# finleygou/GS-MARL

Measured on NVIDIA B200. Metric: agent-steps/sec (graph obs+reward+cost) at 1/2/4/8 B200; % HBM roofline, higher is better.
Workload: dtype f32

## Files before the change

gs_marl_b200/csrc/gsm_kernels_wide.cuh:

```cuda
#pragma once
#include "gsm_kernels_spec.cuh"
#include "gsm_bulk.cuh"

namespace gsm {

constexpr int kWideThreads = 128;
__host__ __device__ constexpr int wide_pow2(int v) { int p = 1; while (p < v) p <<= 1; return p; }

template <typename T, int N, int E>
struct WideConsts {
  T size[E];
  T mass[N], mass_inv[N], accel[N], maxsp[N];
  int32_t eflag[E];
};

#ifndef GSM_WIDE_BLOCKS
#define GSM_WIDE_BLOCKS 7
#endif
template <typename T> struct WideMinBlocks { static constexpr int value = sizeof(T) == 4 ? GSM_WIDE_BLOCKS : 1; };

__device__ __forceinline__ float softplus1(float x) {
  float y, l;
  asm("ex2.approx.ftz.f32 %0, %1;" : "=f"(y) : "f"(-fabsf(x) * 1.4426950408889634f));
  asm("lg2.approx.ftz.f32 %0, %1;" : "=f"(l) : "f"(1.0f + y));
  return fmaxf(x, 0.f) + 0.6931471805599453f * l;
}
__device__ __forceinline__ double softplus1(double x) { return fmax(x, 0.0) + r_log1p(r_exp(-fabs(x))); }

__device__ __forceinline__ int keep(int v) { return __shfl_sync(0xffffffffu, v, threadIdx.x & 31); }
__device__ __forceinline__ unsigned keep(unsigned v) { return __shfl_sync(0xffffffffu, v, threadIdx.x & 31); }
__device__ __forceinline__ float keep(float v) { return __shfl_sync(0xffffffffu, v, threadIdx.x & 31); }
__device__ __forceinline__ double keep(double v) { return __shfl_sync(0xffffffffu, v, threadIdx.x & 31); }

__device__ __forceinline__ void sts(unsigned a, unsigned v) { asm volatile("st.shared.u32 [%0], %1;" :: "r"(a), "r"(v) : "memory"); }
__device__ __forceinline__ void sts(unsigned a, int v) { asm volatile("st.shared.u32 [%0], %1;" :: "r"(a), "r"(v) : "memory"); }
__device__ __forceinline__ void sts(unsigned a, float v) { asm volatile("st.shared.f32 [%0], %1;" :: "r"(a), "f"(v) : "memory"); }
__device__ __forceinline__ void sts(unsigned a, double v) { asm volatile("st.shared.f64 [%0], %1;" :: "r"(a), "d"(v) : "memory"); }
__device__ __forceinline__ void sts2(unsigned a, float x, float y) { asm volatile("st.shared.v2.f32 [%0], {%1, %2};" :: "r"(a), "f"(x), "f"(y) : "memory"); }
__device__ __forceinline__ void sts2(unsigned a, double x, double y) { asm volatile("st.shared.v2.f64 [%0], {%1, %2};" :: "r"(a), "d"(x), "d"(y) : "memory"); }
__device__ __forceinline__ void sts4(unsigned a, float x, float y, float z, float w) {
  asm volatile("st.shared.v4.f32 [%0], {%1, %2, %3, %4};" :: "r"(a), "f"(x), "f"(y), "f"(z), "f"(w) : "memory");
}
__device__ __forceinline__ void sts4(unsigned a, double x, double y, double z, double w) { sts2(a, x, y); sts2(a + 16, z, w); }
__device__ __forceinline__ void lds4(unsigned a, float& x, float& y, float& z, float& w) {
  asm volatile("ld.shared.v4.f32 {%0, %1, %2, %3}, [%4];" : "=f"(x), "=f"(y), "=f"(z), "=f"(w) : "r"(a) : "memory");
}
__device__ __forceinline__ void lds4(unsigned a, double& x, double& y, double& z, double& w) {
  asm volatile("ld.shared.v2.f64 {%0, %1}, [%2];" : "=d"(x), "=d"(y) : "r"(a) : "memory");
  asm volatile("ld.shared.v2.f64 {%0, %1}, [%2];" : "=d"(z), "=d"(w) : "r"(a + 16) : "memory");
}
__device__ __forceinline__ void sts_if(bool on, unsigned a, unsigned v) {
  asm volatile("{ .reg .pred q; setp.ne.u32 q, %2, 0; @q st.shared.u32 [%0], %1; }" :: "r"(a), "r"(v), "r"((unsigned)on) : "memory");
}
__device__ __forceinline__ void sts2_if(bool on, unsigned a, float x, float y) {
  asm volatile("{ .reg .pred q; setp.ne.u32 q, %3, 0; @q st.shared.v2.f32 [%0], {%1, %2}; }" :: "r"(a), "f"(x), "f"(y), "r"((unsigned)on) : "memory");
}
__device__ __forceinline__ void sts2_if(bool on, unsigned a, double x, double y) {
  asm volatile("{ .reg .pred q; setp.ne.u32 q, %3, 0; @q st.shared.v2.f64 [%0], {%1, %2}; }" :: "r"(a), "d"(x), "d"(y), "r"((unsigned)on) : "memory");
}
__device__ __forceinline__ unsigned selp(bool c, unsigned a, unsigned b) {
  unsigned r;
  asm("{ .reg .pred q; setp.ne.u32 q, %3, 0; selp.b32 %0, %1, %2, q; }" : "=r"(r) : "r"(a), "r"(b), "r"((unsigned)c));
  return r;
}
__device__ __forceinline__ float div_eager(float a, float b) {
  float r; asm volatile("div.approx.f32 %0, %1, %2;" : "=f"(r) : "f"(a), "f"(b)); return r;
}
__device__ __forceinline__ double div_eager(double a, double b) { return a / b; }
__device__ __forceinline__ float4 lds16(unsigned a) {
  float4 v; asm volatile("ld.shared.v4.f32 {%0, %1, %2, %3}, [%4];" : "=f"(v.x), "=f"(v.y), "=f"(v.z), "=f"(v.w) : "r"(a) : "memory"); return v;
}

template <typename T>
__device__ __forceinline__ T shfl_xor(T v, int m) { return __shfl_xor_sync(0xffffffffu, v, m); }

template <typename T> struct __align__(16) WideEnt { T x, y, vx, vy; };

struct WideSmem {
  unsigned feat, idx, obs, cnt, adj, cost, rew, asg, buf;
  unsigned ent, warp;
};
__host__ __device__ constexpr WideSmem wide_smem_layout(int rb, int N, int E, int K, int EPW) {
  WideSmem w{};
  unsigned o = 0;
  w.feat = o; o += (unsigned)(EPW * N * K * GSM_NBR_FEAT_DIM * rb);
  w.idx = o; o += ((unsigned)(EPW * N * K * 4) + 15u) & ~15u;
  w.obs = o; o += (unsigned)(EPW * N * GSM_OBS_DIM * rb);
  w.cnt = o; o += (unsigned)(EPW * N * 4);
  w.adj = o; o += (unsigned)(EPW * N * 4);
  w.cost = o; o += (unsigned)(EPW * N * rb);
  w.rew = o; o += (unsigned)(EPW * N * rb);
  w.asg = o; o += (unsigned)(EPW * N * 4);
  w.buf = (o + 15u) & ~15u;
  w.ent = 2 * w.buf;
  w.warp = w.ent + (unsigned)(EPW * E * 4 * rb);
  return w;
}
__host__ __device__ constexpr size_t wide_smem_bytes(int rb, int N, int E, int K, int EPW) {
  return (size_t)(kWideThreads / 32) * wide_smem_layout(rb, N, E, K, EPW).warp;
}

template <typename T, int N, int L, int MODE, int KT>
__global__ void __launch_bounds__(kWideThreads, WideMinBlocks<T>::value)
env_wide_kernel(const __grid_constant__ KParams<T> p, const int n_steps,
                const __grid_constant__ StepStrides ss,
                const __grid_constant__ WideConsts<T, N, N + L> wc,
                const __grid_constant__ WideSmem lay_rt) {
  constexpr int E = N + L, M = E - 1, GW = wide_pow2(M), EPW = 32 / GW;
  constexpr bool OBS = MODE == 1;
  constexpr bool BF = MODE == 2;
  constexpr unsigned FULL = 0xffffffffu;
  constexpr int RB = (int)sizeof(T);
  constexpr int RS4 = EPW * N * 4, RST = EPW * N * RB;
  constexpr int PS = (RS4 % 16 == 0 && RST % 16 == 0) ? 16 : 8;
  constexpr int PC4 = RS4 / PS, PCT = RST / PS, NPIECE = 3 * PC4 + 2 * PCT;
  constexpr bool ROLE_OK = NPIECE <= 32;
  static_assert(GW <= 32 && E <= 32, "an env must fit in one warp, adjacency in one word");
  static_assert(L >= N && 2 * N <= GW + 1 && N >= 3, "goal i is landmark i, held by lane N-1+i; lanes 0..2 stage scalars");
  static_assert(RS4 % 8 == 0 && RST % 8 == 0, "per-warp scalar blocks leave in 8- or 16-byte pieces");
  static_assert(EPW * N * M * 4 / 16 <= 64 && EPW * N * GSM_OBS_DIM * RB / 16 <= 64, "idx / obs blocks leave in <= 2 passes");
  typedef Arith<T> A;
  typedef WideEnt<T> Ent;
  typedef float4 V;
  extern __shared__ __align__(128) unsigned char wsm[];
  const int K = KT > 0 ? KT : p.K;
  const WideSmem lay = KT > 0 ? wide_smem_layout((int)sizeof(T), N, N + L, KT > 0 ? KT : 1, 32 / wide_pow2(N + L - 1)) : lay_rt;
  const int lane = keep((int)(threadIdx.x & 31)), warp = threadIdx.x >> 5;
  const int grp = lane / GW, j = lane % GW, shift = grp * GW;
  const int env_w0 = keep((int)(((int64_t)blockIdx.x * (kWideThreads / 32) + warp) * EPW));
  bool active = env_w0 + grp < p.n_envs;
  if (OBS && p.mask != nullptr && active) active = p.mask[(int64_t)(env_w0 + grp) * p.mask_stride] != 0;
  const int env = active ? env_w0 + grp : 0;
  const bool has = M == GW ? true : j < M;
  const bool own = j < N;
  const int ja = own ? j : 0;
  const unsigned act_bits = __ballot_sync(FULL, active);
  const bool bulk = ROLE_OK && act_bits == FULL && ((EPW * N * K * 4) & 15) == 0 &&
      ((((uintptr_t)p.obs | (uintptr_t)p.nbr_idx | (uintptr_t)p.nbr_feat | (uintptr_t)p.nbr_cnt | (uintptr_t)p.adj |
         (uintptr_t)p.assign | (uintptr_t)p.reward | (uintptr_t)p.cost | (uintptr_t)ss.obs | (uintptr_t)ss.nbr_idx |
         (uintptr_t)ss.nbr_feat | (uintptr_t)ss.nbr_cnt | (uintptr_t)ss.adj | (uintptr_t)ss.assign |
         (uintptr_t)ss.reward | (uintptr_t)ss.cost) & 15) == 0);

  constexpr unsigned ES = (unsigned)sizeof(Ent);
  const unsigned sa_w = keep(smem_u32(wsm) + (unsigned)warp * lay.warp);
  const unsigned sa_ent = keep(smem_u32(wsm) + (unsigned)warp * lay.warp + lay.ent + (unsigned)(grp * E) * ES);

  const int e_hi = has ? j + 1 : 0;
  const int fl_o = wc.eflag[e_hi];
  const T size_o = keep(wc.size[e_hi]), type_o = keep((T)(fl_o >> 1));
  const unsigned lfl = keep((unsigned)((has && (wc.eflag[0] & 1) && (fl_o & 1)) ? 1u : 0u) |
                            ((has && (e_hi < N || (p.cost_obstacles && (fl_o >> 1) == GSM_ENT_OBSTACLE))) ? 2u : 0u) |
                            (((has && p.own_goal_always && j >= N - 1 && j < 2 * N - 1) ? (unsigned)(j - (N - 1) + 1) : 0u) << 8));
  const bool cpair = lfl & 1u, colc = lfl & 2u;
  const int goal_i = (int)(lfl >> 8) - 1;

  T mx = 0, my = 0, mvx = 0, mvy = 0;
  if (active) {
    const T* a = p.agent_state + ((int64_t)env * N + ja) * 4;
    mx = a[0]; my = a[1]; mvx = a[2]; mvy = a[3];
  }
  if (own) sts4(sa_ent + (unsigned)j * ES, mx, my, mvx, mvy);
  if (has && j + 1 >= N) {
    T lx = 0, ly = 0;
    if (active) { const T* l = p.lm_pos + ((int64_t)env * L + (j + 1 - N)) * 2; lx = l[0]; ly = l[1]; }
    sts4(sa_ent + (unsigned)(j + 1) * ES, lx, ly, (T)0, (T)0);
  }
  int t_now = active ? p.t[env] : 0;
  const bool auto_reset = MODE == 2 && p.auto_reset != 0;
  const T accel_m = keep(wc.accel[ja]), mass_m = keep(wc.mass[ja]), massinv_m = keep(wc.mass_inv[ja]), maxsp_m = keep(wc.maxsp[ja]);

  const unsigned char* b_act = (const unsigned char*)p.actions;
  unsigned char* b_obs = (unsigned char*)p.obs;
  unsigned char* b_idx = (unsigned char*)p.nbr_idx;
  unsigned char* b_feat = (unsigned char*)p.nbr_feat;
  unsigned char* b_done = (unsigned char*)p.done;
  const unsigned wrow0 = (unsigned)env_w0 * N;
  unsigned char* c_role = nullptr;
  int64_t role_stride = ss.nbr_cnt;
  {
    const int q = lane;
    if (q < PC4) c_role = (unsigned char*)p.nbr_cnt + wrow0 * 4u + q * PS;
    else if (q < 2 * PC4) { c_role = (unsigned char*)p.adj + wrow0 * 4u + (q - PC4) * PS; if (RB != 4) role_stride = ss.adj; }
    else if (q < 2 * PC4 + PCT) { c_role = (unsigned char*)p.cost + wrow0 * (unsigned)RB + (q - 2 * PC4) * PS; if (RB != 4) role_stride = ss.cost; }
    else if (q < 2 * PC4 + 2 * PCT) { c_role = (unsigned char*)p.reward + wrow0 * (unsigned)RB + (q - 2 * PC4 - PCT) * PS; if (RB != 4) role_stride = ss.reward; }
    else if (q < NPIECE) { c_role = (unsigned char*)p.assign + wrow0 * 4u + (q - 2 * PC4 - 2 * PCT) * PS; if (RB != 4) role_stride = ss.assign; }
  }
  const bool role_on = lane < NPIECE && (!OBS || lane < 2 * PC4 || lane >= 2 * PC4 + 2 * PCT);
  if (own) {
    sts(sa_w + lay.asg + (unsigned)(grp * N + j) * 4u, j);
    sts(sa_w + lay.buf + lay.asg + (unsigned)(grp * N + j) * 4u, j);
  }

  const bool discrete = p.action_mode == GSM_ACT_DISCRETE;
  const unsigned act_off = keep(discrete ? ((unsigned)env * N + ja) * 4u : ((unsigned)env * N + ja) * 2u * (unsigned)RB);
  const unsigned n_idx = (lay.obs - lay.idx) / 16, n_obs = (lay.cnt - lay.obs) / 16;
  const unsigned off_idx = keep(wrow0 * (unsigned)(K * 4) + (unsigned)lane * 16u), off_obs = keep(wrow0 * (unsigned)(GSM_OBS_DIM * RB) + (unsigned)lane * 16u);
  const unsigned off_done = keep((unsigned)env * N + (unsigned)ja);
  int act_next = 0;
  T actx_next = 0, acty_next = 0;
  if (!OBS) {
    if (discrete) act_next = *(const int32_t*)(b_act + act_off);
    else { actx_next = ((const T*)(b_act + act_off))[0]; acty_next = ((const T*)(b_act + act_off))[1]; }
  }
  __syncwarp();

  T fox = 0, foy = 0;
  bool pro = !OBS;
  int step = 0;
  unsigned sb = sa_w;
  int sb_delta = (int)lay.buf;
  const unsigned o_feat = keep((unsigned)(grp * N * K) * (unsigned)(GSM_NBR_FEAT_DIM * RB));
  const unsigned o_idx = keep(lay.idx + (unsigned)(grp * N * K) * 4u);
  const unsigned o_sc = keep(lay.cnt + (unsigned)(j < 3 ? j : 0) * (unsigned)RS4 + (unsigned)(grp * N) * 4u);
  const unsigned o_obs = keep(lay.obs + (unsigned)grp * (unsigned)(N * GSM_OBS_DIM * RB));
  const auto segment_end = [&]() {
    int s = n_steps;
    if (MODE == 2 && auto_reset) {
      const int left = __reduce_min_sync(FULL, active ? p.episode_length - t_now : INT_MAX);
      s = step + max(1, min(left, n_steps - step));
    }
    return s;
  };
  int stop = segment_end();
  while (step < n_steps) {
   for (;;) {
    if (!OBS && !pro) {
      T ux = actx_next, uy = acty_next;
      if (discrete) {
        const int a = act_next;
        ux = 0; uy = 0;
        if (a >= 0 && a < p.n_actions) { ux = p.discrete_u[a][0]; uy = p.discrete_u[a][1]; }
      }
      if (step + 1 < n_steps) b_act += ss.actions;
      if (discrete) act_next = *(const int32_t*)(b_act + act_off);
      else { actx_next = ((const T*)(b_act + act_off))[0]; acty_next = ((const T*)(b_act + act_off))[1]; }
      const T fx = accel_m * ux + fox, fy = accel_m * uy + foy;
      T nvx = mvx * p.one_minus_damp, nvy = mvy * p.one_minus_damp;
      nvx = nvx + A::div_const(fx, mass_m, massinv_m) * p.dt;
      nvy = nvy + A::div_const(fy, mass_m, massinv_m) * p.dt;
      if (maxsp_m > (T)0) {
        const T sp = A::sqrt(nvx * nvx + nvy * nvy);
        if (sp > maxsp_m) { nvx = A::div(nvx, sp) * maxsp_m; nvy = A::div(nvy, sp) * maxsp_m; }
      }
      mvx = nvx; mvy = nvy;
      mx = mx + nvx * p.dt; my = my + nvy * p.dt;
      t_now += 1;
      if (own) sts4(sa_ent + (unsigned)j * ES, mx, my, mvx, mvy);
      __syncwarp();
    }
    const bool st_on = !pro;
    const unsigned a_feat = sb + o_feat, a_idx = sb + o_idx, a_sc = sb + o_sc, sobs = sb + o_obs;
    if (st_on && bulk && lane == 0) bulk_wait_read<1>();

    T fcx[N], fcy[N];
    T gxs = 0, gys = 0, gd = 0;
    bool anyc = false;
#pragma unroll
    for (int i = 0; i < N; i++) {
      const int e = e_hi - (j < i ? 1 : 0);
      Ent si, so;
      lds4(sa_ent + (unsigned)i * ES, si.x, si.y, si.vx, si.vy);
      lds4(sa_ent + (unsigned)e * ES, so.x, so.y, so.vx, so.vy);
      const T dx = so.x - si.x, dy = so.y - si.y;
      const T dist = A::sqrt(dx * dx + dy * dy);
      const T dmin = wc.size[i] + size_o;
      const bool nb = (has && dist < p.Rs) || goal_i == i;
      const bool col = colc && dist < dmin;
      const unsigned bits = (__ballot_sync(FULL, nb) >> shift) & low_mask(GW);
      const unsigned cbits = (__ballot_sync(FULL, col) >> shift) & low_mask(GW);
      int cnt = __popc(bits);
      const int rank = __popc(bits & low_mask(j));
      const int pos = nb ? rank : cnt + (j - rank);
      if (BF) {
        const bool row_on = st_on && has && (KT >= M || pos < K);
        sts_if(row_on, a_idx + (unsigned)pos * 4u + (unsigned)(i * K * 4), (unsigned)(nb ? e : -1));
        const unsigned f = a_feat + (unsigned)pos * (unsigned)(GSM_NBR_FEAT_DIM * RB) + (unsigned)(i * K * GSM_NBR_FEAT_DIM * RB);
        const T z = (T)0;
        sts2_if(row_on, f, nb ? dx : z, nb ? dy : z);
        sts2_if(row_on, f + 2 * RB, nb ? so.vx - si.vx : z, nb ? so.vy - si.vy : z);
        sts2_if(row_on, f + 4 * RB, nb ? dist : z, nb ? type_o : z);
      } else if (has && pos < K && st_on) {
        sts(a_idx + (unsigned)pos * 4u + (unsigned)(i * K * 4), nb ? e : -1);
        const unsigned f = a_feat + (unsigned)pos * (unsigned)(GSM_NBR_FEAT_DIM * RB) + (unsigned)(i * K * GSM_NBR_FEAT_DIM * RB);
        const T z = (T)0;
        if (nb) { sts2(f, dx, dy); sts2(f + 2 * RB, so.vx - si.vx, so.vy - si.vy); sts2(f + 4 * RB, dist, type_o); }
        else { sts2(f, z, z); sts2(f + 2 * RB, z, z); sts2(f + 4 * RB, z, z); }
      }
      if (cnt > K) cnt = K;
      const unsigned ebits = (bits & low_mask(i)) | ((bits & ~low_mask(i)) << 1);
      if (BF && RB == 4) {
        const unsigned v = selp(j == 0, (unsigned)cnt, selp(j == 1, ebits, __float_as_uint((float)__popc(cbits))));
        sts_if(st_on && j < 3, a_sc + (unsigned)(i * 4), v);
      } else if (st_on && j < 3) {
        const unsigned ao = (unsigned)(grp * N + i);
        if (RB == 4) {
          const unsigned v = j == 0 ? (unsigned)cnt : (j == 1 ? ebits : __float_as_uint((float)__popc(cbits)));
          if (!OBS || j < 2) sts(a_sc + (unsigned)(i * 4), v);
        } else {
          if (j == 0) sts(sb + lay.cnt + ao * 4u, cnt);
          else if (j == 1) sts(sb + lay.adj + ao * 4u, ebits);
          else if (!OBS) sts(sb + lay.cost + ao * (unsigned)RB, (T)__popc(cbits));
        }
      }
      if (j == N - 1 + i) { gxs = dx; gys = dy; gd = dist; }
      if (BF) {
        const T x = A::div_const(-(dist - dmin), p.km, p.km_inv);
        const bool term = cpair && !(Prec<T>::kCut && x < (T)(-kFarCut));
        const T pen = softplus1(x) * p.km;
        const T qx = div_eager(p.cf * (-dx), dist), qy = div_eager(p.cf * (-dy), dist);
        fcx[i] = term ? qx * pen : (T)0;
        fcy[i] = term ? qy * pen : (T)0;
        anyc = anyc || term;
      } else if (!OBS) {
        fcx[i] = 0; fcy[i] = 0;
        if (cpair) {
          const T x = A::div_const(-(dist - dmin), p.km, p.km_inv);
          if (!(Prec<T>::kCut && x < (T)(-kFarCut))) {
            const T pen = softplus1(x) * p.km;
            fcx[i] = A::div(p.cf * (-dx), dist) * pen;
            fcy[i] = A::div(p.cf * (-dy), dist) * pen;
            anyc = true;
          }
        }
      }
    }
    if (!OBS && (pro || step + 1 < n_steps)) {
      fox = 0; foy = 0;
      if (__any_sync(FULL, anyc)) {
#pragma unroll
        for (int m = GW / 2; m >= 1; m >>= 1) {
#pragma unroll
          for (int i = 0; i < N; i++) { fcx[i] = fcx[i] + shfl_xor(fcx[i], m); fcy[i] = fcy[i] + shfl_xor(fcy[i], m); }
        }
#pragma unroll
        for (int i = 0; i < N; i++) if (ja == i) { fox = fcx[i]; foy = fcy[i]; }
      }
    }

    if (st_on) {
      if (own) { sts2(sobs + (unsigned)j * (GSM_OBS_DIM * RB), mvx, mvy); sts2(sobs + (unsigned)j * (GSM_OBS_DIM * RB) + 2 * RB, mx, my); }
      T rs = ((T)0 - p.w_dist * gd) + (gd < p.goal_tol ? p.w_goal : (T)0);
      if (p.share_reward && !OBS) {
        T s = shfl(FULL, rs, shift + N - 1);
#pragma unroll
        for (int k = 1; k < N; k++) s = s + shfl(FULL, rs, shift + N - 1 + k);
        rs = s / (T)N;
      }
      if (j >= N - 1 && j < 2 * N - 1) {
        const unsigned ao = (unsigned)(j - (N - 1));
        sts2(sobs + ao * (GSM_OBS_DIM * RB) + 4 * RB, gxs, gys);
        if (!OBS) sts(sb + lay.rew + ((unsigned)grp * N + ao) * (unsigned)RB, rs);
      }
      if (!OBS && own && active) b_done[off_done] = (uint8_t)(t_now >= p.episode_length);
      if (bulk) {
        fence_async_smem();
        __syncwarp();
        if (lane == 0) {
          asm volatile("cp.async.bulk.global.shared::cta.bulk_group [%0], [%1], %2;"
                       :: "l"(b_feat + wrow0 * (unsigned)(K * GSM_NBR_FEAT_DIM * RB)), "r"(sb), "r"(lay.idx) : "memory");
          bulk_commit();
        }
        V* const g_idx = (V*)(b_idx + off_idx);
        V* const g_obs = (V*)(b_obs + off_obs);
        const unsigned s_idx = sb + lay.idx + (unsigned)lane * 16u, s_obs = sb + lay.obs + (unsigned)lane * 16u;
        if (lane < n_idx) g_idx[0] = lds16(s_idx);
        if (lane + 32 < n_idx) g_idx[32] = lds16(s_idx + 512);
        if (lane < n_obs) g_obs[0] = lds16(s_obs);
        if (lane + 32 < n_obs) g_obs[32] = lds16(s_obs + 512);
        if (role_on) {
          if (PS == 16) *(V*)c_role = lds16(sb + lay.cnt + (unsigned)lane * 16u);
          else {
            float2 v8;
            asm volatile("ld.shared.v2.f32 {%0, %1}, [%2];" : "=f"(v8.x), "=f"(v8.y) : "r"(sb + lay.cnt + (unsigned)lane * 8u) : "memory");
            *(float2*)c_role = v8;
          }
        }
      } else {
        __syncwarp();
        auto copy_words = [&](unsigned char* g, unsigned soff, unsigned bytes) {
          const unsigned wpe = bytes / (4 * EPW);
          for (unsigned q = lane; q < bytes / 4; q += 32)
            if ((act_bits >> ((q / wpe) * GW)) & 1u) {
              unsigned v; asm volatile("ld.shared.u32 %0, [%1];" : "=r"(v) : "r"(sb + soff + q * 4u) : "memory");
              ((uint32_t*)g)[q] = v;
            }
        };
        copy_words(b_feat + wrow0 * (unsigned)(K * GSM_NBR_FEAT_DIM * RB), lay.feat, lay.idx - lay.feat);
        copy_words(b_idx + wrow0 * (unsigned)(K * 4), lay.idx, (unsigned)(EPW * N * K * 4));
        copy_words(b_obs + wrow0 * (unsigned)(GSM_OBS_DIM * RB), lay.obs, lay.cnt - lay.obs);
        copy_words((unsigned char*)p.nbr_cnt + (int64_t)step * ss.nbr_cnt + wrow0 * 4u, lay.cnt, RS4);
        copy_words((unsigned char*)p.adj + (int64_t)step * ss.adj + wrow0 * 4u, lay.adj, RS4);
        copy_words((unsigned char*)p.assign + (int64_t)step * ss.assign + wrow0 * 4u, lay.asg, RS4);
        if (!OBS) {
          copy_words((unsigned char*)p.reward + (int64_t)step * ss.reward + wrow0 * (unsigned)RB, lay.rew, RST);
          copy_words((unsigned char*)p.cost + (int64_t)step * ss.cost + wrow0 * (unsigned)RB, lay.cost, RST);
        }
        __syncwarp();
      }
    }
    if (OBS) break;
    if (pro) { pro = false; continue; }
    b_obs += ss.obs; b_idx += ss.nbr_idx; b_feat += ss.nbr_feat; b_done += ss.done;
    c_role += role_stride;
    sb += sb_delta;
    sb_delta = -sb_delta;
    step++;
    if (step >= stop) break;
   }
   if (OBS) break;
   if (MODE == 2 && auto_reset) {
     const bool fin = active && t_now >= p.episode_length;
     if (__any_sync(FULL, fin)) {
       __syncwarp();
       int ep = 0;
       if (fin) {
         const uint64_t genv = (uint64_t)(p.env_offset + env);
         ep = p.episode[env];
#pragma unroll 1
         for (int e = j; e < E; e += GW) {
           double dx, dy;
           spawn_draw_inline(genv, ep, e, p.seed, p.ext[wc.eflag[e] >> 1], dx, dy);
           const T x = (T)dx, y = (T)dy;
           sts4(sa_ent + (unsigned)e * ES, x, y, (T)0, (T)0);
           if (e < N) { mx = x; my = y; }
           else { T* l = p.lm_pos + ((int64_t)env * L + (e - N)) * 2; l[0] = x; l[1] = y; }
         }
         mvx = 0; mvy = 0;
         t_now = 0;
       }
       __syncwarp();
       if (fin && j == 0) p.episode[env] = ep + 1;
       __syncwarp();
       pro = step < n_steps;
       stop = segment_end();
     }
   }
  }
  if (bulk && lane == 0) bulk_wait_read<0>();

  if (!OBS && active) {
    if (own) {
      T* a = p.agent_state + ((int64_t)env * N + j) * 4;
      st2<T>(a, mx, my); st2<T>(a + 2, mvx, mvy);
    }
    if (j == 0) p.t[env] = t_now;
  }
}

}
```

Measured before the change: 16.46 billion.

## Use packed f32x2 arithmetic and streaming cache hints in the BF wide-kernel path

In the BF mode, the velocity and position integration, pairwise deltas, contact-force computation (paired softplus over agents) and the shuffle reductions are rewritten with packed f32x2 add/mul/fma PTX and a scaled rcp-based vector divide. This aims to halve the FP32 instruction count in this path. Global output stores now use evict-first and streaming cache hints, so write-once data is less likely to pollute L2. The divide is now approximate and rounding may change slightly, and the new path needs hardware that supports f32x2 instructions.

```diff
diff --git a/gs_marl_b200/csrc/gsm_kernels_wide.cuh b/gs_marl_b200/csrc/gsm_kernels_wide.cuh
--- a/gs_marl_b200/csrc/gsm_kernels_wide.cuh
+++ b/gs_marl_b200/csrc/gsm_kernels_wide.cuh
@@ -63,10 +63,60 @@
   asm("{ .reg .pred q; setp.ne.u32 q, %3, 0; selp.b32 %0, %1, %2, q; }" : "=r"(r) : "r"(a), "r"(b), "r"((unsigned)c));
   return r;
 }
-__device__ __forceinline__ float div_eager(float a, float b) {
-  float r; asm volatile("div.approx.f32 %0, %1, %2;" : "=f"(r) : "f"(a), "f"(b)); return r;
-}
-__device__ __forceinline__ double div_eager(double a, double b) { return a / b; }
+
+__device__ __forceinline__ float2 bc2(float s) { return make_float2(s, s); }
+__device__ __forceinline__ double2 bc2(double s) { return make_double2(s, s); }
+__device__ __forceinline__ float2 add2(float2 a, float2 b) {
+  float2 r;
+  asm("{ .reg .b64 a, b, d; mov.b64 a, {%2, %3}; mov.b64 b, {%4, %5}; add.rn.f32x2 d, a, b; mov.b64 {%0, %1}, d; }"
+      : "=f"(r.x), "=f"(r.y) : "f"(a.x), "f"(a.y), "f"(b.x), "f"(b.y));
+  return r;
+}
+__device__ __forceinline__ float2 sub2(float2 a, float2 b) {
+  float2 r;
+  asm("{ .reg .b64 a, b, d; mov.b64 a, {%2, %3}; mov.b64 b, {%4, %5}; sub.rn.f32x2 d, a, b; mov.b64 {%0, %1}, d; }"
+      : "=f"(r.x), "=f"(r.y) : "f"(a.x), "f"(a.y), "f"(b.x), "f"(b.y));
+  return r;
+}
+__device__ __forceinline__ float2 mul2(float2 a, float2 b) {
+  float2 r;
+  asm("{ .reg .b64 a, b, d; mov.b64 a, {%2, %3}; mov.b64 b, {%4, %5}; mul.rn.f32x2 d, a, b; mov.b64 {%0, %1}, d; }"
+      : "=f"(r.x), "=f"(r.y) : "f"(a.x), "f"(a.y), "f"(b.x), "f"(b.y));
+  return r;
+}
+__device__ __forceinline__ float2 fma2(float2 a, float2 b, float2 c) {
+  float2 r;
+  asm("{ .reg .b64 a, b, c, d; mov.b64 a, {%2, %3}; mov.b64 b, {%4, %5}; mov.b64 c, {%6, %7}; fma.rn.f32x2 d, a, b, c; mov.b64 {%0, %1}, d; }"
+      : "=f"(r.x), "=f"(r.y) : "f"(a.x), "f"(a.y), "f"(b.x), "f"(b.y), "f"(c.x), "f"(c.y));
+  return r;
+}
+__device__ __forceinline__ double2 add2(double2 a, double2 b) { return make_double2(a.x + b.x, a.y + b.y); }
+__device__ __forceinline__ double2 sub2(double2 a, double2 b) { return make_double2(a.x - b.x, a.y - b.y); }
+__device__ __forceinline__ double2 mul2(double2 a, double2 b) { return make_double2(a.x * b.x, a.y * b.y); }
+__device__ __forceinline__ double2 fma2(double2 a, double2 b, double2 c) { return make_double2(a.x * b.x + c.x, a.y * b.y + c.y); }
+__device__ __forceinline__ float2 div2(float2 a, float b) {
+  float2 r;
+  asm("{ .reg .pred p; .reg .f32 b, t; .reg .b64 a, d;\n\t"
+      "mov.b64 a, {%2, %3}; abs.f32 t, %4; setp.lt.f32 p, t, 0f00800000; selp.f32 t, 0f4B800000, 0f3F800000, p;\n\t"
+      "mul.rn.f32 b, %4, t; mov.b64 d, {t, t}; mul.rn.f32x2 a, a, d;\n\t"
+      "rcp.approx.ftz.f32 t, b; mov.b64 d, {t, t}; mul.rn.f32x2 d, a, d; mov.b64 {%0, %1}, d; }"
+      : "=f"(r.x), "=f"(r.y) : "f"(a.x), "f"(a.y), "f"(b));
+  return r;
+}
+__device__ __forceinline__ double2 div2(double2 a, double b) { return make_double2(a.x / b, a.y / b); }
+__device__ __forceinline__ double2 softplus2(double2 x) { return make_double2(softplus1(x.x), softplus1(x.y)); }
+__device__ __forceinline__ float2 softplus2(float2 x) {
+  float2 y, l;
+  asm("ex2.approx.ftz.f32 %0, %1;" : "=f"(y.x) : "f"(-fabsf(x.x) * 1.4426950408889634f));
+  asm("ex2.approx.ftz.f32 %0, %1;" : "=f"(y.y) : "f"(-fabsf(x.y) * 1.4426950408889634f));
+  y = add2(bc2(1.0f), y);
+  asm("lg2.approx.ftz.f32 %0, %1;" : "=f"(l.x) : "f"(y.x));
+  asm("lg2.approx.ftz.f32 %0, %1;" : "=f"(l.y) : "f"(y.y));
+  return fma2(bc2(0.6931471805599453f), l, make_float2(fmaxf(x.x, 0.f), fmaxf(x.y, 0.f)));
+}
+__device__ __forceinline__ float2 div_const2(float2 a, float , float b_inv) { return mul2(a, bc2(b_inv)); }
+__device__ __forceinline__ double2 div_const2(double2 a, double b, double ) { return make_double2(a.x / b, a.y / b); }
+
 __device__ __forceinline__ float4 lds16(unsigned a) {
   float4 v; asm volatile("ld.shared.v4.f32 {%0, %1, %2, %3}, [%4];" : "=f"(v.x), "=f"(v.y), "=f"(v.z), "=f"(v.w) : "r"(a) : "memory"); return v;
 }
@@ -120,6 +170,7 @@
   static_assert(RS4 % 8 == 0 && RST % 8 == 0, "per-warp scalar blocks leave in 8- or 16-byte pieces");
   static_assert(EPW * N * M * 4 / 16 <= 64 && EPW * N * GSM_OBS_DIM * RB / 16 <= 64, "idx / obs blocks leave in <= 2 passes");
   typedef Arith<T> A;
+  typedef typename Vec2<T>::type T2;
   typedef WideEnt<T> Ent;
   typedef float4 V;
   extern __shared__ __align__(128) unsigned char wsm[];
@@ -234,16 +285,28 @@
       if (step + 1 < n_steps) b_act += ss.actions;
       if (discrete) act_next = *(const int32_t*)(b_act + act_off);
       else { actx_next = ((const T*)(b_act + act_off))[0]; acty_next = ((const T*)(b_act + act_off))[1]; }
-      const T fx = accel_m * ux + fox, fy = accel_m * uy + foy;
-      T nvx = mvx * p.one_minus_damp, nvy = mvy * p.one_minus_damp;
-      nvx = nvx + A::div_const(fx, mass_m, massinv_m) * p.dt;
-      nvy = nvy + A::div_const(fy, mass_m, massinv_m) * p.dt;
-      if (maxsp_m > (T)0) {
-        const T sp = A::sqrt(nvx * nvx + nvy * nvy);
-        if (sp > maxsp_m) { nvx = A::div(nvx, sp) * maxsp_m; nvy = A::div(nvy, sp) * maxsp_m; }
-      }
-      mvx = nvx; mvy = nvy;
-      mx = mx + nvx * p.dt; my = my + nvy * p.dt;
+      if (BF) {
+        const T2 f = fma2(bc2(accel_m), T2{ux, uy}, T2{fox, foy});
+        T2 nv = fma2(T2{mvx, mvy}, bc2(p.one_minus_damp), mul2(div_const2(f, mass_m, massinv_m), bc2(p.dt)));
+        if (maxsp_m > (T)0) {
+          const T sp = A::sqrt(nv.x * nv.x + nv.y * nv.y);
+          if (sp > maxsp_m) nv = mul2(div2(nv, sp), bc2(maxsp_m));
+        }
+        mvx = nv.x; mvy = nv.y;
+        const T2 np = fma2(nv, bc2(p.dt), T2{mx, my});
+        mx = np.x; my = np.y;
+      } else {
+        const T fx = accel_m * ux + fox, fy = accel_m * uy + foy;
+        T nvx = mvx * p.one_minus_damp, nvy = mvy * p.one_minus_damp;
+        nvx = nvx + A::div_const(fx, mass_m, massinv_m) * p.dt;
+        nvy = nvy + A::div_const(fy, mass_m, massinv_m) * p.dt;
+        if (maxsp_m > (T)0) {
+          const T sp = A::sqrt(nvx * nvx + nvy * nvy);
+          if (sp > maxsp_m) { nvx = A::div(nvx, sp) * maxsp_m; nvy = A::div(nvy, sp) * maxsp_m; }
+        }
+        mvx = nvx; mvy = nvy;
+        mx = mx + nvx * p.dt; my = my + nvy * p.dt;
+      }
       t_now += 1;
       if (own) sts4(sa_ent + (unsigned)j * ES, mx, my, mvx, mvy);
       __syncwarp();
@@ -255,13 +318,16 @@
     T fcx[N], fcy[N];
     T gxs = 0, gys = 0, gd = 0;
     bool anyc = false;
+    T2 cd[N];
+    T cdist[N], cdmin[N];
 #pragma unroll
     for (int i = 0; i < N; i++) {
       const int e = e_hi - (j < i ? 1 : 0);
       Ent si, so;
       lds4(sa_ent + (unsigned)i * ES, si.x, si.y, si.vx, si.vy);
       lds4(sa_ent + (unsigned)e * ES, so.x, so.y, so.vx, so.vy);
-      const T dx = so.x - si.x, dy = so.y - si.y;
+      const T2 d = BF ? sub2(T2{so.x, so.y}, T2{si.x, si.y}) : T2{so.x - si.x, so.y - si.y};
+      const T dx = d.x, dy = d.y;
       const T dist = A::sqrt(dx * dx + dy * dy);
       const T dmin = wc.size[i] + size_o;
       const bool nb = (has && dist < p.Rs) || goal_i == i;
@@ -276,8 +342,9 @@
         sts_if(row_on, a_idx + (unsigned)pos * 4u + (unsigned)(i * K * 4), (unsigned)(nb ? e : -1));
         const unsigned f = a_feat + (unsigned)pos * (unsigned)(GSM_NBR_FEAT_DIM * RB) + (unsigned)(i * K * GSM_NBR_FEAT_DIM * RB);
         const T z = (T)0;
+        const T2 dv = sub2(T2{so.vx, so.vy}, T2{si.vx, si.vy});
         sts2_if(row_on, f, nb ? dx : z, nb ? dy : z);
-        sts2_if(row_on, f + 2 * RB, nb ? so.vx - si.vx : z, nb ? so.vy - si.vy : z);
+        sts2_if(row_on, f + 2 * RB, nb ? dv.x : z, nb ? dv.y : z);
         sts2_if(row_on, f + 4 * RB, nb ? dist : z, nb ? type_o : z);
       } else if (has && pos < K && st_on) {
         sts(a_idx + (unsigned)pos * 4u + (unsigned)(i * K * 4), nb ? e : -1);
@@ -304,13 +371,23 @@
       }
       if (j == N - 1 + i) { gxs = dx; gys = dy; gd = dist; }
       if (BF) {
-        const T x = A::div_const(-(dist - dmin), p.km, p.km_inv);
-        const bool term = cpair && !(Prec<T>::kCut && x < (T)(-kFarCut));
-        const T pen = softplus1(x) * p.km;
-        const T qx = div_eager(p.cf * (-dx), dist), qy = div_eager(p.cf * (-dy), dist);
-        fcx[i] = term ? qx * pen : (T)0;
-        fcy[i] = term ? qy * pen : (T)0;
-        anyc = anyc || term;
+        cd[i] = d; cdist[i] = dist; cdmin[i] = dmin;
+        const auto contact = [&](int c, T x, T pen) {
+          const bool term = cpair && !(Prec<T>::kCut && x < (T)(-kFarCut));
+          const T2 fc = mul2(div2(mul2(cd[c], bc2(-p.cf)), cdist[c]), bc2(pen));
+          fcx[c] = term ? fc.x : (T)0;
+          fcy[c] = term ? fc.y : (T)0;
+          anyc = anyc || term;
+        };
+        if (i % 2 == 1) {
+          const T2 x = div_const2(sub2(T2{cdist[i - 1], dist}, T2{cdmin[i - 1], dmin}), -p.km, -p.km_inv);
+          const T2 pen = mul2(softplus2(x), bc2(p.km));
+          contact(i - 1, x.x, pen.x);
+          contact(i, x.y, pen.y);
+        } else if (i == N - 1) {
+          const T x = A::div_const(-(dist - dmin), p.km, p.km_inv);
+          contact(i, x, softplus1(x) * p.km);
+        }
       } else if (!OBS) {
         fcx[i] = 0; fcy[i] = 0;
         if (cpair) {
@@ -325,15 +402,29 @@
       }
     }
     if (!OBS && (pro || step + 1 < n_steps)) {
-      fox = 0; foy = 0;
+      if (!BF) { fox = 0; foy = 0; }
       if (__any_sync(FULL, anyc)) {
 #pragma unroll
         for (int m = GW / 2; m >= 1; m >>= 1) {
 #pragma unroll
-          for (int i = 0; i < N; i++) { fcx[i] = fcx[i] + shfl_xor(fcx[i], m); fcy[i] = fcy[i] + shfl_xor(fcy[i], m); }
-        }
+          for (int i = 0; i < N; i++) {
+            if (BF) {
+              const T2 s = add2(T2{fcx[i], fcy[i]}, T2{shfl_xor(fcx[i], m), shfl_xor(fcy[i], m)});
+              fcx[i] = s.x; fcy[i] = s.y;
+            } else {
+              fcx[i] = fcx[i] + shfl_xor(fcx[i], m); fcy[i] = fcy[i] + shfl_xor(fcy[i], m);
+            }
+          }
+        }
+        if (!BF) {
 #pragma unroll
-        for (int i = 0; i < N; i++) if (ja == i) { fox = fcx[i]; foy = fcy[i]; }
+          for (int i = 0; i < N; i++) if (ja == i) { fox = fcx[i]; foy = fcy[i]; }
+        }
+      }
+      if (BF) {
+        fox = fcx[N - 1]; foy = fcy[N - 1];
+#pragma unroll
+        for (int i = 0; i < N - 1; i++) if (j == i) { fox = fcx[i]; foy = fcy[i]; }
       }
     }
 
@@ -356,19 +447,26 @@
         fence_async_smem();
         __syncwarp();
         if (lane == 0) {
-          asm volatile("cp.async.bulk.global.shared::cta.bulk_group [%0], [%1], %2;"
-                       :: "l"(b_feat + wrow0 * (unsigned)(K * GSM_NBR_FEAT_DIM * RB)), "r"(sb), "r"(lay.idx) : "memory");
+          unsigned char* const g_feat = b_feat + wrow0 * (unsigned)(K * GSM_NBR_FEAT_DIM * RB);
+          if (BF)
+            asm volatile("{ .reg .b64 pol; createpolicy.fractional.L2::evict_first.b64 pol, 1.0;\n\t"
+                         "cp.async.bulk.global.shared::cta.bulk_group.L2::cache_hint [%0], [%1], %2, pol; }"
+                         :: "l"(g_feat), "r"(sb), "r"(lay.idx) : "memory");
+          else
+            asm volatile("cp.async.bulk.global.shared::cta.bulk_group [%0], [%1], %2;"
+                         :: "l"(g_feat), "r"(sb), "r"(lay.idx) : "memory");
           bulk_commit();
         }
         V* const g_idx = (V*)(b_idx + off_idx);
         V* const g_obs = (V*)(b_obs + off_obs);
         const unsigned s_idx = sb + lay.idx + (unsigned)lane * 16u, s_obs = sb + lay.obs + (unsigned)lane * 16u;
-        if (lane < n_idx) g_idx[0] = lds16(s_idx);
-        if (lane + 32 < n_idx) g_idx[32] = lds16(s_idx + 512);
-        if (lane < n_obs) g_obs[0] = lds16(s_obs);
-        if (lane + 32 < n_obs) g_obs[32] = lds16(s_obs + 512);
+        const auto put16 = [&](V* g, const V v) { if (BF) __stcs(g, v); else *g = v; };
+        if (lane < n_idx) put16(g_idx, lds16(s_idx));
+        if (lane + 32 < n_idx) put16(g_idx + 32, lds16(s_idx + 512));
+        if (lane < n_obs) put16(g_obs, lds16(s_obs));
+        if (lane + 32 < n_obs) put16(g_obs + 32, lds16(s_obs + 512));
         if (role_on) {
-          if (PS == 16) *(V*)c_role = lds16(sb + lay.cnt + (unsigned)lane * 16u);
+          if (PS == 16) put16((V*)c_role, lds16(sb + lay.cnt + (unsigned)lane * 16u));
           else {
             float2 v8;
             asm volatile("ld.shared.v2.f32 {%0, %1}, [%2];" : "=f"(v8.x), "=f"(v8.y) : "r"(sb + lay.cnt + (unsigned)lane * 8u) : "memory");
```

Result: faster. 17.08 billion (median of 6 runs) (+3.8%).
